# sp-uhh/sgmse

Measured on AMD Instinct MI355X. Metric: utterances/sec, SGMSE+ NCSN++ PC N=30 (reverse_diffusion + ALD, 60 NFE), 16 kHz 4 s utterances, higher is better.
Workload: dtype f32 (fp16x2-split products, fp32 accumulate); 1 GPU; BASELINE configs[1]: ncsnpp (65.6M params) PC sampler N=30, batch=32 x 4 s @16 kHz per GPU, hipGraph-captured step; batch_per_gpu=32, F=256, T=512, nfe=60, sampler=pc, parallelism=utterance-sharded x1 (weights broadcast once over RCCL)

## Files before the change

### include/sgmse_hip.h

```cpp
#ifndef SGMSE_HIP_H
#define SGMSE_HIP_H

#ifdef __cplusplus
extern "C" {
#endif

typedef struct sgmse_ctx sgmse_ctx;

typedef enum { SGMSE_OK = 0, SGMSE_EINVAL = -1, SGMSE_ERUNTIME = -2, SGMSE_ENOTREADY = -3 } sgmse_status;

typedef struct {
  int variant;
  int nf;
  int n_levels;
  int ch_mult[8];
  int num_res_blocks;
  int n_attn;
  int attn_res[8];
  int image_size;
  int progressive;
  int progressive_input;
  int scale_by_sigma;
} sgmse_net_cfg;

// ... 36 lines not shown
int sgmse_stft(sgmse_ctx* ctx, const float* sig, const float* window, void* spec, int B, int L, int n_fft, int hop);
int sgmse_istft(sgmse_ctx* ctx, const void* spec, const float* window, float* out, int B, int K, int n_fft, int hop,
                int length);
int sgmse_spec_fwd(sgmse_ctx* ctx, const void* in, void* out, long long n, int transform_type, float factor, float exponent);
int sgmse_spec_back(sgmse_ctx* ctx, const void* in, void* out, long long n, int transform_type, float factor, float exponent);

int sgmse_upfirdn2d(sgmse_ctx* ctx, const float* input, const float* kernel, float* out, int BC, int H, int W, int kh,
                    int kw, int up_x, int up_y, int down_x, int down_y, int pad_x0, int pad_x1, int pad_y0, int pad_y1);
int sgmse_upfirdn2d_dtype(sgmse_ctx* ctx, int dtype, const void* input, const void* kernel, void* out, int BC, int H, int W,
                          int kh, int kw, int up_x, int up_y, int down_x, int down_y, int pad_x0, int pad_x1, int pad_y0,
                          int pad_y1);

int sgmse_op_conv2d(sgmse_ctx* ctx, const float* x, const float* w_oihw, const float* bias, const float* res, float* out,
                    int B, int Cin, int Cout, int H, int W, int ks, float out_scale, int force_direct,
                    const float* in_scale, const float* in_shift, int in_act, const float* x2, int C2);
int sgmse_op_groupnorm(sgmse_ctx* ctx, const float* x, const float* gamma, const float* beta, float* out, int B, int C,
                       int H, int W, int act, const float* x2, int C2);
int sgmse_op_fir(sgmse_ctx* ctx, const float* x, float* out, int BC, int H, int W, int up, const float* in_scale,
                 const float* in_shift, int in_act, float* out_raw);
int sgmse_op_attention(sgmse_ctx* ctx, const float* qkv, float* out, int B, int C, int S);

int sgmse_conv_split_mode(sgmse_ctx* ctx, int* out);
int sgmse_conv_winograd(sgmse_ctx* ctx, int* out);

#define SGMSE_NCLASS 8
int sgmse_profile_forward(sgmse_ctx* ctx, const void* xy, const float* t, void* out, int B, int F, int T, float* ms,
                          double* work, int* launches);
int sgmse_bench_conv(sgmse_ctx* ctx, int ks, int B, int Cin, int Cout, int H, int W, int variant, int iters, int fused,
                     float* ms);
int sgmse_calib_stream(sgmse_ctx* ctx, int mode, int bytes_per_lane, long long total_bytes, float* ms);
// ... 11 lines not shown
```

### sgmse_amd/_lib.py

```python
from __future__ import annotations

import ctypes as C
import os
import threading
from typing import Dict, Optional, Sequence

import torch

_HERE = os.path.dirname(os.path.abspath(__file__))
DEFAULT_LIB = os.path.join(_HERE, "libsgmse_hip.so")

SGMSE_NCLASS = 8
CLASS_NAMES = ("conv3x3_wide", "conv3x3_other", "conv1x1", "conv_direct", "groupnorm_stats", "fir",
               "attention", "entry_exit")
CLASS_WORK_UNIT = ("flop", "flop", "flop", "flop", "byte", "byte", "flop", "byte")


class NetCfgC(C.Structure):
    _fields_ = [("variant", C.c_int), ("nf", C.c_int), ("n_levels", C.c_int), ("ch_mult", C.c_int * 8),
                ("num_res_blocks", C.c_int), ("n_attn", C.c_int), ("attn_res", C.c_int * 8), ("image_size", C.c_int),
                ("progressive", C.c_int), ("progressive_input", C.c_int), ("scale_by_sigma", C.c_int)]


class SamplerCfgC(C.Structure):
# ... 17 lines not shown
    "sgmse_last_error": (C.c_char_p, [_P]),
    "sgmse_backend": (C.c_char_p, []),
    "sgmse_configure": (_I, [_P, C.POINTER(NetCfgC)]),
    "sgmse_load_weights": (_I, [_P, C.POINTER(C.c_char_p), C.POINTER(_P), C.POINTER(_LL), _I, _I]),
    "sgmse_param_count": (_I, [_P, C.POINTER(_LL)]),
    "sgmse_ncsnpp_forward": (_I, [_P, _P, _P, _P, _I, _I, _I]),
    "sgmse_pc_sample": (_I, [_P, _P, _P, _I, _I, _I, C.POINTER(SamplerCfgC), _P, C.c_ulonglong, C.POINTER(_I)]),
    "sgmse_sb_sample": (_I, [_P, _P, _P, _I, _I, _I, _I] + [C.POINTER(_F)] * 8 + [_I, _P, C.c_ulonglong, _I, C.POINTER(_I)]),
    "sgmse_stft": (_I, [_P, _P, _P, _P, _I, _I, _I, _I]),
    "sgmse_istft": (_I, [_P, _P, _P, _P, _I, _I, _I, _I, _I]),
    "sgmse_spec_fwd": (_I, [_P, _P, _P, _LL, _I, _F, _F]),
    "sgmse_spec_back": (_I, [_P, _P, _P, _LL, _I, _F, _F]),
    "sgmse_upfirdn2d": (_I, [_P, _P, _P, _P] + [_I] * 13),
    "sgmse_upfirdn2d_dtype": (_I, [_P, _I, _P, _P, _P] + [_I] * 13),
    "sgmse_op_conv2d": (_I, [_P, _P, _P, _P, _P, _P, _I, _I, _I, _I, _I, _I, _F, _I, _P, _P, _I, _P, _I]),
    "sgmse_op_groupnorm": (_I, [_P, _P, _P, _P, _P, _I, _I, _I, _I, _I, _P, _I]),
    "sgmse_conv_split_mode": (_I, [_P, _P]),
    "sgmse_conv_winograd": (_I, [_P, _P]),
    "sgmse_op_fir": (_I, [_P, _P, _P, _I, _I, _I, _I, _P, _P, _I, _P]),
    "sgmse_op_attention": (_I, [_P, _P, _P, _I, _I, _I]),
    "sgmse_profile_forward": (_I, [_P, _P, _P, _P, _I, _I, _I, C.POINTER(_F), C.POINTER(C.c_double), C.POINTER(_I)]),
    "sgmse_bench_conv": (_I, [_P, _I, _I, _I, _I, _I, _I, _I, _I, _I, C.POINTER(_F)]),
    "sgmse_calib_stream": (_I, [_P, _I, _I, C.c_longlong, C.POINTER(_F)]),
    "sgmse_arena_bytes": (_I, [_P, C.POINTER(_LL)]),
    "sgmse_graph_captures": (_I, [_P, C.POINTER(_I)]),
    "sgmse_graph_updates": (_I, [_P, C.POINTER(_I)]),
    "sgmse_set_noise_streams": (_I, [_P, C.POINTER(C.c_ulonglong), _I]),
    "sgmse_set_frames": (_I, [_P, C.POINTER(_I), _I]),
}
EXPORTED_SYMBOLS = tuple(_SIGS)
# ... 384 lines not shown
```

### sgmse_amd/csrc/capi.h

```cpp
#pragma once
#include <string>
#include "engine.h"
#include "../../include/sgmse_hip.h"

struct sgmse_ctx {
  sgmse::Engine* eng = nullptr;
  std::string err;
};

namespace {
template <class Fn>
int sg_guard(sgmse_ctx* ctx, Fn&& fn) {
  if (!ctx || !ctx->eng) return SGMSE_EINVAL;
  try {
    fn(*ctx->eng);
    return SGMSE_OK;
  } catch (const sgmse::EngineError& e) {
    ctx->err = e.what();
    const bool notready = ctx->err.find("weights not loaded") != std::string::npos;
    return notready ? SGMSE_ENOTREADY : SGMSE_ERUNTIME;
  } catch (const std::exception& e) {
    ctx->err = std::string("internal error: ") + e.what();
    return SGMSE_ERUNTIME;
  }
// ... 130 lines not shown
  SG_ARG(ctx, up_x >= 1 && up_y >= 1 && down_x >= 1 && down_y >= 1, "up/down factors must be >= 1");
  return sg_guard(ctx, [&](sgmse::Engine& e) { e.op_upfirdn2d(dtype, input, kernel, out, BC, H, W, kh, kw, up_x, up_y, down_x, down_y, px0, px1, py0, py1); });
}

int sgmse_op_conv2d(sgmse_ctx* ctx, const float* x, const float* w, const float* bias, const float* res, float* out, int B, int Cin,
                    int Cout, int H, int W, int ks, float out_scale, int force_direct, const float* in_scale,
                    const float* in_shift, int in_act, const float* x2, int C2) {
  SG_ARG(ctx, x && w && out && B > 0 && Cin > 0 && Cout > 0 && H > 0 && W > 0, "null pointer or non-positive shape");
  SG_ARG(ctx, ks == 1 || ks == 3, "kernel size must be 1 or 3");
  SG_ARG(ctx, (x2 == nullptr) == (C2 == 0) && C2 >= 0 && C2 < Cin, "bad second source");
  return sg_guard(ctx, [&](sgmse::Engine& e) {
    e.op_conv2d(x, w, bias, res, out, B, Cin, Cout, H, W, ks, out_scale, force_direct, in_scale, in_shift, in_act, x2, C2);
  });
}

int sgmse_op_groupnorm(sgmse_ctx* ctx, const float* x, const float* gamma, const float* beta, float* out, int B, int C, int H,
                       int W, int act, const float* x2, int C2) {
  SG_ARG(ctx, x && gamma && beta && out && B > 0 && C >= 4 && H > 0 && W > 0, "null pointer or non-positive shape");
  SG_ARG(ctx, C % (C / 4 < 32 ? C / 4 : 32) == 0, "C must be divisible by min(C/4, 32)");
  return sg_guard(ctx, [&](sgmse::Engine& e) { e.op_groupnorm(x, gamma, beta, out, B, C, H, W, act, x2, C2); });
}

int sgmse_conv_split_mode(sgmse_ctx* ctx, int* out) {
  SG_ARG(ctx, out != nullptr, "out is null");
  return sg_guard(ctx, [&](sgmse::Engine& e) { *out = e.split_mode(); });
}

int sgmse_conv_winograd(sgmse_ctx* ctx, int* out) {
  SG_ARG(ctx, out != nullptr, "out is null");
  return sg_guard(ctx, [&](sgmse::Engine& e) { *out = e.winograd() ? 1 : 0; });
// ... 56 lines not shown
```

### sgmse_amd/csrc/conv_launch.h

```cpp
#pragma once
#include "conv_route.h"
#include "kernels_conv.h"
#include "kernels_conv_pipe.h"
#include "kernels_conv1x1.h"
#include "kernels_conv_split.h"
#include "kernels_conv_wino.h"
#include "kernels_conv_wino43.h"
#include "kernels_conv_wino2d.h"
#include "kernels_conv_thin.h"

#ifndef SGMSE_CONV_SPLIT_DEFAULT
#define SGMSE_CONV_SPLIT_DEFAULT 2
#endif
#ifndef SGMSE_CONV_PIPE_DEFAULT
#define SGMSE_CONV_PIPE_DEFAULT 1
#endif

namespace sgmse {

inline int conv_variant() {
  static int v = [] { const char* e = getenv("SGMSE_CONV_VARIANT"); return e ? atoi(e) : 0; }();
  return v;
}

// ... 101 lines not shown
  if (abl && mode == 2) {
#define SGMSE_ABL_CASE(V) if (abl == V) { DRT_LAUNCH((conv3x3_split_kernel<SplitH2, 0, 1, V>), grid, dim3(256), st, a); return; }
#ifdef SGMSE_ABLATION_FULL
    SGMSE_ABL_CASE(8) SGMSE_ABL_CASE(59) SGMSE_ABL_CASE(64)
    SGMSE_ABL_CASE(3) SGMSE_ABL_CASE(4) SGMSE_ABL_CASE(24) SGMSE_ABL_CASE(56)
    SGMSE_ABL_CASE(1) SGMSE_ABL_CASE(2) SGMSE_ABL_CASE(67) SGMSE_ABL_CASE(72) SGMSE_ABL_CASE(128) SGMSE_ABL_CASE(256) SGMSE_ABL_CASE(512)
#endif
#undef SGMSE_ABL_CASE
  }
  if (mode == 2) launch_conv3x3_split_t<SplitH2, 0>(a, grid, st); else launch_conv3x3_split_t<SplitB3, 0>(a, grid, st);
}

inline bool conv_wino43_aligned(const ConvArgs& a) {
  return reinterpret_cast<uintptr_t>(a.src1) % 16 == 0 && (a.src2 == nullptr || reinterpret_cast<uintptr_t>(a.src2) % 16 == 0);
}
template <int ROWS>
inline void launch_conv_wino_rows(WinoForm form, const ConvArgs& a, drt::stream_t st) {
  const dim3 grid(conv_grid_tiles(a, ROWS), a.Cout / 128, 1);
  const bool act = a.in_scale && a.in_act;
  if (form == WinoForm::F43) {
    if (act) DRT_LAUNCH((conv3x3_wino43_kernel<ROWS, 1>), grid, dim3(512), st, a);
    else DRT_LAUNCH((conv3x3_wino43_kernel<ROWS, 0>), grid, dim3(512), st, a);
  } else {
    if (a.sc_w) DRT_LAUNCH((conv3x3_wino_kernel<ROWS, 1, 1>), grid, dim3(512), st, a);
    else if (act) DRT_LAUNCH((conv3x3_wino_kernel<ROWS, 1, 0>), grid, dim3(512), st, a);
    else DRT_LAUNCH((conv3x3_wino_kernel<ROWS, 0, 0>), grid, dim3(512), st, a);
  }
}
inline void launch_conv_wino(WinoForm form, const ConvArgs& a, drt::stream_t st, bool rows4, bool trace = false, int abl = 0) {
  if (form == WinoForm::F2x2) {
    const dim3 grid(conv_grid_tiles(a, 4), a.Cout / 128, 1);
    if (abl == 8) DRT_LAUNCH((conv3x3_wino2d_kernel<1, 8>), grid, dim3(512), st, a);
    else if (abl == 16) DRT_LAUNCH((conv3x3_wino2d_kernel<1, 16>), grid, dim3(512), st, a);
    else if (a.in_scale && a.in_act) DRT_LAUNCH((conv3x3_wino2d_kernel<1>), grid, dim3(512), st, a);
    else DRT_LAUNCH((conv3x3_wino2d_kernel<0>), grid, dim3(512), st, a);
    return;
  }
#ifdef SGMSE_ABLATION_FULL
  const dim3 grid8(conv_grid_tiles(a, 8), a.Cout / 128, 1);
  if (form == WinoForm::F43) {
    if (trace) { DRT_LAUNCH((conv3x3_wino43_kernel<8, 1, 1>), grid8, dim3(512), st, a); return; }
  } else {
#define SGMSE_WABL_CASE(V) if (abl == V) { DRT_LAUNCH((conv3x3_wino_kernel<8, 1, 0, 0, V>), grid8, dim3(512), st, a); return; }
    SGMSE_WABL_CASE(1) SGMSE_WABL_CASE(2) SGMSE_WABL_CASE(4) SGMSE_WABL_CASE(8) SGMSE_WABL_CASE(16) SGMSE_WABL_CASE(24) SGMSE_WABL_CASE(3) SGMSE_WABL_CASE(32) SGMSE_WABL_CASE(20)
#undef SGMSE_WABL_CASE
    if (trace) { DRT_LAUNCH((conv3x3_wino_kernel<8, 1, 0, 1>), grid8, dim3(512), st, a); return; }
  }
#endif
  (void)abl; (void)trace;
  if (rows4) launch_conv_wino_rows<4>(form, a, st); else launch_conv_wino_rows<8>(form, a, st);
}

inline void launch_conv_thin(const ConvArgs& a, drt::stream_t st) {
  const dim3 grid(conv_thin_grid_tiles(a, (a.W + ConvThinGeom::TW - 1) / ConvThinGeom::TW), 1, 1);
  if (a.in_scale && a.in_act) DRT_LAUNCH((conv3x3_thin_kernel<1>), grid, dim3(256), st, a);
  else DRT_LAUNCH((conv3x3_thin_kernel<0>), grid, dim3(256), st, a);
}

inline void launch_conv_direct(const ConvArgs& a, int ks, drt::stream_t st) {
  const int HW = a.H * a.W;
  if (a.Cout <= 4) {
    dim3 grid((HW + 255) / 256, 1, a.B);
    if (ks == 3) DRT_LAUNCH((conv_direct_kernel<3, 4>), grid, dim3(256), st, a);
    else DRT_LAUNCH((conv_direct_kernel<1, 4>), grid, dim3(256), st, a);
  } else {
// ... 8 lines not shown
```

### sgmse_amd/csrc/engine.h

```cpp
#pragma once
#include <map>
#include <string>
#include <vector>
#include <cstdio>
#include <stdexcept>

#include <deque>
#include <sgmse_devrt.h>
#include "kernels_conv.h"
#include "conv_launch.h"
#include "kernels_norm_fir.h"
#include "kernels_attn_misc.h"
#include "kernels_stft.h"

namespace sgmse {

struct EngineError : std::runtime_error { using std::runtime_error::runtime_error; };

#define SG_CHECK(expr) do { int _e = (expr); if (_e != 0) { char _b[256]; snprintf(_b, sizeof _b, "%s failed: %s (%d)", #expr, drt::error_string(_e), _e); throw EngineError(_b); } } while (0)
#define SG_REQUIRE(cond, msg) do { if (!(cond)) throw EngineError(std::string(msg)); } while (0)

struct NetCfg {
  int variant = 0;
  int nf = 128;
// ... 550 lines not shown
      if (bounds) free_tmp(bounds);
      if (xb) free_tmp(xb);
    } else if (pl.mfma && !force_direct && (C2 == 0 || a.C1 % ((ks == 3) ? 8 : 32) == 0)) {
      const float* pk = pack_mfma(oihw_sources(w_oihw, ks, Cin, Cout), pl.co_t, false);
      a.w = pk;
      launch_conv_mfma(a, ks, pl, stream_);
      SG_CHECK(drt::stream_sync(stream_));
      free_tmp(const_cast<float*>(pk));
    } else {
      a.w = w_oihw;
      launch_conv_direct(a, ks, stream_);
    }
    check_launch();
  }

  void op_groupnorm(const float* x, const float* gamma, const float* beta, float* out, int B, int C, int H, int W, int act,
                    const float* x2, int C2) {
    const int HW = H * W, C1 = C - C2;
    float* stats = static_cast<float*>(dev_alloc_tmp((size_t)B * C * 2 * 4));
    float* sc = static_cast<float*>(dev_alloc_tmp((size_t)B * C * 4));
    float* sh = static_cast<float*>(dev_alloc_tmp((size_t)B * C * 4));
    float* stats2 = stats + (size_t)B * C1 * 2;
    DRT_LAUNCH(gn_chan_stats_kernel, dim3(B * C1), dim3(256), stream_, x, (const float*)nullptr, C1, 0, HW, stats, Rag{nullptr, nullptr, nullptr}, 0);
    if (C2) DRT_LAUNCH(gn_chan_stats_kernel, dim3(B * C2), dim3(256), stream_, x2, (const float*)nullptr, C2, 0, HW, stats2, Rag{nullptr, nullptr, nullptr}, 0);
    const int G = std::min(C / 4, 32);
    const GnFin f{stats, stats2, nullptr, nullptr, gamma, beta, sc, sh, nullptr, Rag{nullptr, nullptr, nullptr}, C1, 1, 1, C2, 1, 1, G, HW, 0, 1e-6f};
    DRT_LAUNCH(gn_finalize_kernel, dim3(G, B), dim3(256), stream_, f);
    DRT_LAUNCH(gn_apply_kernel, dim3((HW + 1023) / 1024, B * C), dim3(256), stream_, x, x2, C1, C2, HW, (const float*)sc,
               (const float*)sh, act, out);
    SG_CHECK(drt::stream_sync(stream_));
// ... 45 lines not shown
  }

  void op_spec_xform(const float2* in, float2* out, size_t n, int type, float factor, float exponent, int inverse) {
    SpecXformArgs a{in, out, n, type, factor, exponent, inverse};
    DRT_LAUNCH(spec_xform_kernel, dim3((unsigned)((n + 255) / 256)), dim3(256), stream_, a);
    check_launch();
  }

  void sync() { SG_CHECK(drt::stream_sync(stream_)); }

  float bench_conv(int ks, int B, int Cin, int Cout, int H, int W, int variant, int iters, int fused) {
    ConvPlan pl = choose_conv_plan(ks, Cin, Cout, H, W);
    SG_REQUIRE(pl.mfma, "bench_conv: shape is not MFMA-eligible");
    if (variant >= 0 && (variant & 512)) { pl.rows = 4; variant &= ~512; }
    int ablate = 0, abl_split = 0;
    bool split_rows4 = false, wino43 = false;
    if (variant >= 0) {
      split_rows4 = (variant >> 23) & 1;
      wino43 = (variant >> 22) & 1;
      abl_split = (variant >> 12) & 1023;
      if (!(variant & (64 | 128))) { ablate = abl_split & 15; abl_split = 0; }
      variant &= 4095;
    }
    const bool wino = variant >= 0 && (variant & 1024);
    const bool wino2d = variant >= 0 && (variant & 2048) && !wino;
    const int smode = variant < 0 ? 0 : ((variant & 128) ? 2 : ((variant & 64) ? 1 : 0));
    const bool b3 = smode != 0 && !wino && !wino2d;
    SG_REQUIRE(!(wino || wino2d) || (ks == 3 && conv_wino_eligible(Cin, 0, Cout, W)), "bench_conv: shape is not eligible for the Winograd kernel");
    SG_REQUIRE(!b3 || conv_split_eligible(ks, Cin, 0, Cout), "bench_conv: shape is not eligible for the split kernels");
    wino43 = wino43 && wino;
    SG_REQUIRE(!wino43 || conv_wino43_eligible(Cin, 0, Cout, W), "bench_conv: shape is not eligible for the Winograd F(4,3) kernel");
    const WinoForm wform = wino2d ? WinoForm::F2x2 : wino43 ? WinoForm::F43 : WinoForm::F23;
// ... 24 lines not shown
          a.in_scale = nullptr; a.in_shift = nullptr; a.in_act = 0;
          a.amax1 = bounds;
        } else {
          xbound = producer_bound(a.in_scale, a.in_shift, Cin, bounds, nullptr, B); a.xbound = xbound;
        }
      }
    }
    unsigned long long* trace_dev = nullptr;
    const size_t n_wg = (size_t)B * ((H + 7) / 8) * ((W + 31) / 32) * ((Cout + 127) / 128);
    if (abl_split & 64) {
      trace_dev = static_cast<unsigned long long*>(dev_alloc_tmp(n_wg * 256));
      SG_CHECK(drt::memset_dev(trace_dev, 0, n_wg * 256, stream_));
      a.trace = trace_dev;
    }
    auto go = [&]() {
      if (wino || wino2d) launch_conv_wino(wform, a, stream_, split_rows4, (abl_split & 64) != 0, abl_split & 63);
      else if (b3) launch_conv_split(a, ks, smode, stream_, split_rows4, abl_split);
      else launch_conv_mfma(a, ks, pl, stream_, variant);
    };
    for (int i = 0; i < 2; ++i) go();
    drt::event_record(&e0, stream_);
    for (int i = 0; i < iters; ++i) go();
    drt::event_record(&e1, stream_);
    drt::event_sync(&e1);
    const float ms = drt::event_elapsed_ms(e0, e1) / (float)iters;
    check_launch();
    drt::event_destroy(&e0); drt::event_destroy(&e1);
    if (trace_dev) {
      const size_t words = wino ? 32 : 16;
      std::vector<unsigned long long> h(n_wg * words);
      SG_CHECK(drt::memcpy_d2h(h.data(), trace_dev, n_wg * words * 8, stream_));
// ... 1044 lines not shown
```

### sgmse_amd/csrc/kernels_conv_wino43.h

```cpp
#pragma once
#include "kernels_conv_wino.h"

namespace sgmse {

template <int ROWS_>
struct Wino43Geom {
  static constexpr int KC = 16, ROWS = ROWS_, TROWS = ROWS_ + 2, NF = ROWS_ / 4, NK = 6;
  static constexpr int PV = 25;
  static constexpr int ROW_V = 8 * PV;
  static constexpr int STAGE_V = TROWS * ROW_V;
  static constexpr int NSROW = 4 * TROWS;
  static constexpr int NPASS = (NSROW + 5) / 6;
  static constexpr int CO_V = 512;
  static constexpr int NDIR = ROWS_ == 4 ? 1 : 2;
  static constexpr int XCH_V = 4 * NDIR * 16 * 64;
  static constexpr int LDS_V = (2 * STAGE_V + CO_V) > XCH_V ? (2 * STAGE_V + CO_V) : XCH_V;
  static_assert(NPASS <= 8, "one staging pass per wave");
};

inline size_t packed_wino43_frags(int cin, int cout) { return (size_t)((cout + 127) / 128) * (cin / 16) * 18 * 2 * 4 * 64; }
inline size_t packed_wino43_bytes(int cin, int cout) { return packed_wino43_frags(cin, cout) * 16 + (size_t)((cout + 127) / 128) * 128 * 4; }

__device__ __forceinline__ double wino43_u(double g0, double g1, double g2, int k) {
  return k == 0 ? 0.25 * g0 : k == 1 ? -(g0 + g1 + g2) / 6.0 : k == 2 ? -(g0 - g1 + g2) / 6.0
// ... 42 lines not shown
      double u = 0.0;
      if (co < p.cout) {
        const float* g = p.src + (((size_t)co * p.cin + c) * 3 + dy) * 3;
        u = wino43_u(g[0], g[1], g[2], k);
      }
      u *= ws;
      const uint32_t hi = drt_f32_to_f16((float)u);
      const uint32_t lo = drt_f32_to_f16((float)(u - (double)drt_f16_to_f32(hi)));
      part[h] = split ? lo : hi;
    }
    o[q] = part[0] | (part[1] << 16);
  }
  reinterpret_cast<u32x4*>(p.dst)[e] = o;
}

template <int ROWS, int ACT, int TRACE = 0>
__global__ __launch_bounds__(512, 1) void conv3x3_wino43_kernel(ConvArgs p) {
  using G = Wino43Geom<ROWS>;
  using T = WinoTile<ROWS>;
  using S = SplitH2;
  constexpr int NF = G::NF, PV = G::PV, NS = 2;
  __shared__ u32x4 s_all[G::LDS_V];
  u32x4* const s_in0 = s_all;
  u32x4* const s_in1 = s_all + G::STAGE_V;
  f32x4* const s_co = reinterpret_cast<f32x4*>(s_all + 2 * G::STAGE_V);

  const int tid = threadIdx.x;
  const int wave = drt_uniform(tid >> 6), lane = tid & 63, l31 = lane & 31, kg = lane >> 5;
  const int cf = wave & 3, kh = wave >> 2;
  unsigned long long* trace = nullptr;
  if constexpr (TRACE) {
// ... 162 lines not shown
  if (it_run) {
#pragma unroll
    for (int c = 0; c < 4; ++c) stage_chan_co(c, s_co[4 * it_q + c]);
    flush_item(s_in0);
    load_item((nst > 1 ? 1 : 0) * G::KC);
  }
  __syncthreads();

  if constexpr (TRACE) { if (trace) trace[2] = drt_clock(); }
  constexpr int AR = 3, AD = AR - 1, NTAP = 9;
  unsigned long long tbar = 0, ttap[NTAP] = {0, 0, 0, 0, 0, 0, 0, 0, 0};
  const bool tracer = TRACE && p.trace && (tid == 0 || tid == 256);
  u32x4 ar[AR][NS];
#pragma unroll
  for (int t = 0; t < AD; ++t) load_a(0, t, ar[t]);
#pragma unroll 1
  for (int st = 0; st < nst; ++st) {
    const int stn = st + 1 < nst ? st + 1 : st;
    const int stl = st + 2 < nst ? st + 2 : nst - 1;
    const u32x4* cur = (st & 1) ? s_in1 : s_in0;
    u32x4* nxt = (st & 1) ? s_in0 : s_in1;
#pragma unroll
    for (int tap = 0; tap < NTAP; ++tap) {
      unsigned long long tc0 = 0;
      if constexpr (TRACE) tc0 = drt_clock();
      const int ntap = (tap + AD) % NTAP;
      const int nstg = tap + AD < NTAP ? st : stn;
      load_a(nstg, ntap, ar[(tap + AD) % AR]);
      __builtin_amdgcn_sched_barrier(0);
      const bool ca = tap < 2, cb = tap >= NTAP - 2;
      const int phase = ca ? tap : cb ? tap - (NTAP - 2) : -1;
      const bool stage_here = phase >= 0 && it_run && (ca ? kh == 0 : kh == 1) && st + 1 < nst;
      compute_tap(cur, tap, ar[tap % AR], phase, stage_here, stn * G::KC, nxt);
      if (phase == 1 && stage_here && st + 2 < nst) load_item(stl * G::KC);
      if constexpr (TRACE) { __builtin_amdgcn_sched_barrier(0); ttap[tap] += drt_clock() - tc0; }
    }
    if constexpr (TRACE) {
      const unsigned long long tb = drt_clock();
      __syncthreads();
      tbar += drt_clock() - tb;
    } else {
      __syncthreads();
    }
  }
  if constexpr (TRACE) {
    if (trace) { trace[3] = drt_clock(); trace[6] = tbar; }
    if (tracer) {
      unsigned long long* tq = p.trace + 32 * (size_t)(blockIdx.y * gridDim.x + blockIdx.x) + (tid == 0 ? 11 : 21);
#pragma unroll
      for (int i = 0; i < NTAP; ++i) tq[i] = ttap[i];
      tq[NTAP] = tbar;
    }
  }

  constexpr bool ALL_TO_A = ROWS == 4;
  const bool fin_wave = !ALL_TO_A || kh == 0;
  const int ef = ALL_TO_A ? 0 : kh;
  int tid_e = (int)threadIdx.x;
  DRT_PIN_INT(tid_e);
  const int lane_e = tid_e & 63, l31_e = lane_e & 31, kg_e = lane_e >> 5;
  const int yy_raw = y0 + 4 * ef + (l31_e >> 3), x = x0 + 4 * (l31_e & 7);
  const bool okc = x < W;
  const bool inside = x0 + 32 <= W && y0 + ROWS <= H;
  const size_t ubase = (size_t)b * p.Cout * HW;
  const int co_l = co_blk * 128 + cf * 32 + 4 * kg_e;
  const int yy = yy_raw < H ? yy_raw : H - 1;
  const unsigned lane_boff = (((unsigned)co_l * (unsigned)H + (unsigned)yy) * (unsigned)W + (unsigned)(okc ? x : 0)) * 4u;
  auto soff = [&](int r) -> unsigned { return (unsigned)((r & 3) + 8 * (r >> 2)) * HW * 4u; };
  const drt_buf obuf = drt_make_buf(p.out + ubase), rbuf = drt_make_buf(p.res ? p.res + ubase : p.out);
  const bool has_res = p.res != nullptr;
  float2 rr[16][2];
  if (fin_wave && has_res) {
#pragma unroll
    for (int r = 0; r < 16; ++r) { rr[r][0] = drt_buf_load2(rbuf, lane_boff, soff(r)); rr[r][1] = drt_buf_load2(rbuf, lane_boff + 8u, soff(r)); }
  }
  if constexpr (TRACE) { if (trace) trace[7] = drt_clock() - trace[3]; }
  float yv[4][16];
  {
    float4* xs = reinterpret_cast<float4*>(s_all);
    auto slot = [&](int dir, int r) -> float4* { return xs + (((cf * G::NDIR + dir) * 16 + r) * 64 + lane_e); };
    auto part_a = [&](int f, int r) -> float4 {
      const float m1 = acc[1][f][r], m2 = acc[2][f][r];
      const float sp = m1 + m2, sm = m1 - m2;
      return make_float4(acc[0][f][r] + sp, sm, sp, sm);
    };
    auto part_b = [&](int f, int r) -> float4 {
      const float m3 = acc[0][f][r], m4 = acc[1][f][r];
      const float s = m3 + m4, t = m3 - m4;
      return make_float4(s, 2.f * t, 4.f * s, 8.f * t + acc[2][f][r]);
    };
    if (kh == 0) {
// ... 25 lines not shown
      }
    }
  }
  if constexpr (TRACE) { if (trace) trace[5] = drt_clock() - trace[3]; }
  auto finish = [&](auto guard_tag) {
    constexpr bool GUARD = decltype(guard_tag)::value;
    float cs_inv[16];
    load_cs(cs_inv);
    float s1[16], s2[16], vmax = 0.f;
    const bool ok = !GUARD || (okc && yy_raw < H);
#pragma unroll
    for (int r = 0; r < 16; ++r) {
      float v[4];
#pragma unroll
      for (int i = 0; i < 4; ++i) v[i] = yv[i][r] * cs_inv[r] * inv_kx;
      if (has_res) { v[0] += rr[r][0].x; v[1] += rr[r][0].y; v[2] += rr[r][1].x; v[3] += rr[r][1].y; }
#pragma unroll
      for (int i = 0; i < 4; ++i) v[i] *= p.out_scale;
      if (ok) {
        drt_buf_store2(obuf, make_float2(v[0], v[1]), lane_boff, soff(r));
        drt_buf_store2(obuf, make_float2(v[2], v[3]), lane_boff + 8u, soff(r));
      }
      if (GUARD) {
#pragma unroll
        for (int i = 0; i < 4; ++i) v[i] = ok ? v[i] : 0.f;
      }
      vmax = fmaxf(fmaxf(vmax, fmaxf(fabsf(v[0]), fabsf(v[1]))), fmaxf(fabsf(v[2]), fabsf(v[3])));
      s1[r] = (v[0] + v[1]) + (v[2] + v[3]);
      s2[r] = (v[0] * v[0] + v[1] * v[1]) + (v[2] * v[2] + v[3] * v[3]);
    }
    DRT_PIN_HERE(vmax);
    if constexpr (TRACE) { if (trace) trace[10] = drt_clock() - trace[3]; }
    if (p.stats_out && y0 + 4 * ef < H) {
      auto butterfly = [&](float (&sv)[16]) -> float {
        float a[8];
#pragma unroll
// ... 28 lines not shown
```

### sgmse_amd/csrc/sgmse_devrt.h

```cpp
#pragma once
#include <hip/hip_runtime.h>
#include <cstdint>
#include <cstddef>
#include <cstdlib>
#include <cstring>
#include <cmath>
#include <algorithm>

typedef float f32x16 __attribute__((ext_vector_type(16)));
typedef float f32x4 __attribute__((ext_vector_type(4)));
typedef float f32x2 __attribute__((ext_vector_type(2)));
typedef uint32_t u32x4 __attribute__((ext_vector_type(4)));

__device__ __forceinline__ f32x16 mfma_32x32x16_bf16(u32x4 a, u32x4 b, f32x16 c) {
  typedef __bf16 bf16x8 __attribute__((ext_vector_type(8)));
  return __builtin_amdgcn_mfma_f32_32x32x16_bf16(__builtin_bit_cast(bf16x8, a), __builtin_bit_cast(bf16x8, b), c, 0, 0, 0);
}

__device__ __forceinline__ f32x16 mfma_32x32x16_f16(u32x4 a, u32x4 b, f32x16 c) {
  typedef _Float16 f16x8 __attribute__((ext_vector_type(8)));
  return __builtin_amdgcn_mfma_f32_32x32x16_f16(__builtin_bit_cast(f16x8, a), __builtin_bit_cast(f16x8, b), c, 0, 0, 0);
}
__device__ __forceinline__ uint32_t drt_f32_to_f16(float x) { return (uint32_t)__builtin_bit_cast(uint16_t, (_Float16)x); }
__device__ __forceinline__ float drt_f16_to_f32(uint32_t h) { return (float)__builtin_bit_cast(_Float16, (uint16_t)h); }
// ... 18 lines not shown
}
template <int AUX = 0>
__device__ __forceinline__ void drt_buf_store(const drt_buf& b, float v, unsigned voff, unsigned soff) {
  __builtin_amdgcn_raw_buffer_store_b32(__builtin_bit_cast(unsigned, v), b.r, voff, soff, AUX);
}
template <int AUX = 0>
__device__ __forceinline__ float2 drt_buf_load2(const drt_buf& b, unsigned voff, unsigned soff) {
  const auto v = __builtin_amdgcn_raw_buffer_load_b64(b.r, voff, soff, AUX);
  return make_float2(__builtin_bit_cast(float, (unsigned)v[0]), __builtin_bit_cast(float, (unsigned)v[1]));
}
template <int AUX = 0>
__device__ __forceinline__ void drt_buf_store2(const drt_buf& b, float2 v, unsigned voff, unsigned soff) {
  typedef unsigned u2_t __attribute__((ext_vector_type(2)));
  const u2_t u = {__builtin_bit_cast(unsigned, v.x), __builtin_bit_cast(unsigned, v.y)};
  __builtin_amdgcn_raw_buffer_store_b64(u, b.r, voff, soff, AUX);
}
__device__ __forceinline__ unsigned long long drt_clock() { return __builtin_amdgcn_s_memtime(); }
__device__ __forceinline__ unsigned drt_hw_id() { return __builtin_amdgcn_s_getreg((31 << 11) | 4); }
__device__ __forceinline__ unsigned drt_xcc_id() { return __builtin_amdgcn_s_getreg((31 << 11) | 20); }
__device__ __forceinline__ void drt_atomic_max_nonneg(float* p, float v) {
  atomicMax(reinterpret_cast<unsigned int*>(p), __builtin_bit_cast(unsigned int, v));
}

__device__ __forceinline__ double drt_shfl_xor_f64(double v, int mask) {
  const unsigned long long u = __builtin_bit_cast(unsigned long long, v);
  const unsigned lo = (unsigned)__shfl_xor((int)(unsigned)(u & 0xffffffffull), mask);
  const unsigned hi = (unsigned)__shfl_xor((int)(unsigned)(u >> 32), mask);
  return __builtin_bit_cast(double, ((unsigned long long)hi << 32) | lo);
}

// ... 106 lines not shown
```

### sgmse_amd/ops.py

```python
from __future__ import annotations

from typing import Dict, Optional, Tuple

import torch

from . import _lib

_ctx: Dict[str, "_lib.Context"] = {}


def default_context(device: "torch.device | str | None" = None) -> "_lib.Context":
    if device is None:
        device = "cpu" if _lib.is_emulator() else torch.device("cuda", torch.cuda.current_device())
    key = str(torch.device(device))
    if key not in _ctx:
        _ctx[key] = _lib.Context(device)
    return _ctx[key]


def _f32(t: Optional[torch.Tensor], name: str, dev) -> Optional[torch.Tensor]:
    return None if t is None else _lib.check_tensor(t, name, torch.float32, dev)


def conv2d(x: torch.Tensor, weight: torch.Tensor, bias: Optional[torch.Tensor] = None, *,
# ... 6 lines not shown
    B, C1, H, W = x.shape
    C2 = 0 if x2 is None else x2.shape[1]
    Cout, Cin, kh, kw = weight.shape
    if kh != kw or kh not in (1, 3):
        raise ValueError("kernel must be 1x1 or 3x3")
    if Cin != C1 + C2:
        raise ValueError(f"weight expects {Cin} input channels, got {C1}+{C2}")
    out = torch.empty((B, Cout, H, W), dtype=torch.float32, device=dev)
    ctx.use_current_stream()
    ctx.check(ctx.lib.sgmse_op_conv2d(ctx.h, x.data_ptr(), weight.data_ptr(), _lib.ptr(_f32(bias, "bias", dev)),
                                      _lib.ptr(_f32(residual, "residual", dev)), out.data_ptr(), B, Cin, Cout, H, W, kh,
                                      float(out_scale), {None: int(force_direct), 'bf16x3': 2, 'fp16x2': 3, 'wino': 4, 'wino4': 5, 'thin': 6, 'wino2d': 7, 'wino43': 8, 'wino43_4': 9}[force_split], _lib.ptr(_f32(in_scale, "in_scale", dev)),
                                      _lib.ptr(_f32(in_shift, "in_shift", dev)), int(in_act),
                                      _lib.ptr(_f32(x2, "x2", dev)), C2))
    return out


def group_norm(x: torch.Tensor, weight: torch.Tensor, bias: torch.Tensor, *, act: bool = False,
               x2: Optional[torch.Tensor] = None) -> torch.Tensor:
    ctx = default_context(x.device)
    dev = ctx.device
    x = _f32(x, "x", dev)
    B, C1, H, W = x.shape
    C2 = 0 if x2 is None else x2.shape[1]
    C = C1 + C2
    out = torch.empty((B, C, H, W), dtype=torch.float32, device=dev)
    ctx.use_current_stream()
    ctx.check(ctx.lib.sgmse_op_groupnorm(ctx.h, x.data_ptr(), _f32(weight, "weight", dev).data_ptr(),
                                         _f32(bias, "bias", dev).data_ptr(), out.data_ptr(), B, C, H, W, int(act),
                                         _lib.ptr(_f32(x2, "x2", dev)), C2))
# ... 96 lines not shown
```

Measured before the change: 6.140 utterances/s.

## Overlap Winograd F(4,3) residual loads with last stage and widen epilogue stores

Peels the last K-stage of the Winograd F(4,3) conv main loop so that residual loads are issued during its later taps, hiding their latency behind the MFMA work instead of loading after the loop. The epilogue now loads and stores 128-bit values when output and residual are 16-byte aligned, replacing pairs of 64-bit buffer ops. The old path stays available as the EPI8 template variant and is used as a fallback for unaligned cases. It also adds a standalone op and C API for testing the kernel. Holding the residual in 16 float4 registers during the last stage raises register pressure, which could hurt the schedule.

```diff
diff --git a/include/sgmse_hip.h b/include/sgmse_hip.h
--- a/include/sgmse_hip.h
+++ b/include/sgmse_hip.h
@@ -74,6 +74,9 @@
 int sgmse_op_conv2d(sgmse_ctx* ctx, const float* x, const float* w_oihw, const float* bias, const float* res, float* out,
                     int B, int Cin, int Cout, int H, int W, int ks, float out_scale, int force_direct,
                     const float* in_scale, const float* in_shift, int in_act, const float* x2, int C2);
+int sgmse_op_conv_wino43(sgmse_ctx* ctx, const float* x, const float* w_oihw, const float* bias, const float* res, float* out,
+                         float* stats_out, float* amax_out, const float* xbound, int B, int Cin, int Cout, int H, int W, float out_scale,
+                         const float* in_scale, const float* in_shift, int in_act, const int* frames, int rows4, int epi8);
 int sgmse_op_groupnorm(sgmse_ctx* ctx, const float* x, const float* gamma, const float* beta, float* out, int B, int C,
                        int H, int W, int act, const float* x2, int C2);
 int sgmse_op_fir(sgmse_ctx* ctx, const float* x, float* out, int BC, int H, int W, int up, const float* in_scale,
diff --git a/sgmse_amd/_lib.py b/sgmse_amd/_lib.py
--- a/sgmse_amd/_lib.py
+++ b/sgmse_amd/_lib.py
@@ -55,6 +55,7 @@
     "sgmse_upfirdn2d": (_I, [_P, _P, _P, _P] + [_I] * 13),
     "sgmse_upfirdn2d_dtype": (_I, [_P, _I, _P, _P, _P] + [_I] * 13),
     "sgmse_op_conv2d": (_I, [_P, _P, _P, _P, _P, _P, _I, _I, _I, _I, _I, _I, _F, _I, _P, _P, _I, _P, _I]),
+    "sgmse_op_conv_wino43": (_I, [_P] * 9 + [_I] * 5 + [_F, _P, _P, _I, _P, _I, _I]),
     "sgmse_op_groupnorm": (_I, [_P, _P, _P, _P, _P, _I, _I, _I, _I, _I, _P, _I]),
     "sgmse_conv_split_mode": (_I, [_P, _P]),
     "sgmse_conv_winograd": (_I, [_P, _P]),
diff --git a/sgmse_amd/csrc/capi.h b/sgmse_amd/csrc/capi.h
--- a/sgmse_amd/csrc/capi.h
+++ b/sgmse_amd/csrc/capi.h
@@ -168,6 +168,16 @@
   });
 }
 
+int sgmse_op_conv_wino43(sgmse_ctx* ctx, const float* x, const float* w, const float* bias, const float* res, float* out, float* stats_out,
+                         float* amax_out, const float* xbound, int B, int Cin, int Cout, int H, int W, float out_scale,
+                         const float* in_scale, const float* in_shift, int in_act, const int* frames, int rows4, int epi8) {
+  SG_ARG(ctx, x && w && out && stats_out && amax_out && xbound && B > 0 && Cin > 0 && Cout > 0 && H > 0 && W > 0, "null pointer or non-positive shape");
+  SG_ARG(ctx, (in_scale == nullptr) == (in_shift == nullptr), "in_scale and in_shift come together");
+  return sg_guard(ctx, [&](sgmse::Engine& e) {
+    e.op_conv_wino43(x, w, bias, res, out, stats_out, amax_out, xbound, B, Cin, Cout, H, W, out_scale, in_scale, in_shift, in_act, frames, rows4, epi8);
+  });
+}
+
 int sgmse_op_groupnorm(sgmse_ctx* ctx, const float* x, const float* gamma, const float* beta, float* out, int B, int C, int H,
                        int W, int act, const float* x2, int C2) {
   SG_ARG(ctx, x && gamma && beta && out && B > 0 && C >= 4 && H > 0 && W > 0, "null pointer or non-positive shape");
diff --git a/sgmse_amd/csrc/conv_launch.h b/sgmse_amd/csrc/conv_launch.h
--- a/sgmse_amd/csrc/conv_launch.h
+++ b/sgmse_amd/csrc/conv_launch.h
@@ -139,20 +139,29 @@
 inline bool conv_wino43_aligned(const ConvArgs& a) {
   return reinterpret_cast<uintptr_t>(a.src1) % 16 == 0 && (a.src2 == nullptr || reinterpret_cast<uintptr_t>(a.src2) % 16 == 0);
 }
+inline bool conv_wino43_epilogue_aligned(const ConvArgs& a) {
+  return reinterpret_cast<uintptr_t>(a.out) % 16 == 0 && (a.res == nullptr || reinterpret_cast<uintptr_t>(a.res) % 16 == 0) &&
+         (a.rag_w ? a.rag_vec_ok != 0 : a.W % 4 == 0);
+}
 template <int ROWS>
-inline void launch_conv_wino_rows(WinoForm form, const ConvArgs& a, drt::stream_t st) {
+inline void launch_conv_wino_rows(WinoForm form, const ConvArgs& a, drt::stream_t st, bool epi8) {
   const dim3 grid(conv_grid_tiles(a, ROWS), a.Cout / 128, 1);
   const bool act = a.in_scale && a.in_act;
   if (form == WinoForm::F43) {
-    if (act) DRT_LAUNCH((conv3x3_wino43_kernel<ROWS, 1>), grid, dim3(512), st, a);
-    else DRT_LAUNCH((conv3x3_wino43_kernel<ROWS, 0>), grid, dim3(512), st, a);
+    if (epi8 || !conv_wino43_epilogue_aligned(a)) {
+      if (act) DRT_LAUNCH((conv3x3_wino43_kernel<ROWS, 1, 0, 1>), grid, dim3(512), st, a);
+      else DRT_LAUNCH((conv3x3_wino43_kernel<ROWS, 0, 0, 1>), grid, dim3(512), st, a);
+    } else {
+      if (act) DRT_LAUNCH((conv3x3_wino43_kernel<ROWS, 1>), grid, dim3(512), st, a);
+      else DRT_LAUNCH((conv3x3_wino43_kernel<ROWS, 0>), grid, dim3(512), st, a);
+    }
   } else {
     if (a.sc_w) DRT_LAUNCH((conv3x3_wino_kernel<ROWS, 1, 1>), grid, dim3(512), st, a);
     else if (act) DRT_LAUNCH((conv3x3_wino_kernel<ROWS, 1, 0>), grid, dim3(512), st, a);
     else DRT_LAUNCH((conv3x3_wino_kernel<ROWS, 0, 0>), grid, dim3(512), st, a);
   }
 }
-inline void launch_conv_wino(WinoForm form, const ConvArgs& a, drt::stream_t st, bool rows4, bool trace = false, int abl = 0) {
+inline void launch_conv_wino(WinoForm form, const ConvArgs& a, drt::stream_t st, bool rows4, bool trace = false, int abl = 0, bool epi8 = false) {
   if (form == WinoForm::F2x2) {
     const dim3 grid(conv_grid_tiles(a, 4), a.Cout / 128, 1);
     if (abl == 8) DRT_LAUNCH((conv3x3_wino2d_kernel<1, 8>), grid, dim3(512), st, a);
@@ -164,6 +173,7 @@
 #ifdef SGMSE_ABLATION_FULL
   const dim3 grid8(conv_grid_tiles(a, 8), a.Cout / 128, 1);
   if (form == WinoForm::F43) {
+    if (trace && epi8) { DRT_LAUNCH((conv3x3_wino43_kernel<8, 1, 1, 1>), grid8, dim3(512), st, a); return; }
     if (trace) { DRT_LAUNCH((conv3x3_wino43_kernel<8, 1, 1>), grid8, dim3(512), st, a); return; }
   } else {
 #define SGMSE_WABL_CASE(V) if (abl == V) { DRT_LAUNCH((conv3x3_wino_kernel<8, 1, 0, 0, V>), grid8, dim3(512), st, a); return; }
@@ -173,7 +183,7 @@
   }
 #endif
   (void)abl; (void)trace;
-  if (rows4) launch_conv_wino_rows<4>(form, a, st); else launch_conv_wino_rows<8>(form, a, st);
+  if (rows4) launch_conv_wino_rows<4>(form, a, st, epi8); else launch_conv_wino_rows<8>(form, a, st, epi8);
 }
 
 inline void launch_conv_thin(const ConvArgs& a, drt::stream_t st) {
diff --git a/sgmse_amd/csrc/engine.h b/sgmse_amd/csrc/engine.h
--- a/sgmse_amd/csrc/engine.h
+++ b/sgmse_amd/csrc/engine.h
@@ -588,6 +588,48 @@
     check_launch();
   }
 
+  void op_conv_wino43(const float* x, const float* w_oihw, const float* bias, const float* res, float* out, float* stats_out, float* amax_out,
+                      const float* xbound, int B, int Cin, int Cout, int H, int W, float out_scale, const float* in_scale, const float* in_shift,
+                      int in_act, const int* frames, int rows4, int epi8) {
+    ConvArgs a{};
+    a.src1 = x; a.C1 = Cin; a.bias = bias; a.res = res; a.out_scale = out_scale; a.out = out; a.Cout = Cout; a.B = B; a.H = H; a.W = W;
+    a.in_scale = in_scale; a.in_shift = in_shift; a.in_act = in_act; a.xbound = xbound;
+    SG_REQUIRE(conv_wino43_eligible(Cin, 0, Cout, W) && conv_wino43_aligned(a), "op_conv_wino43: shape is not eligible for the Winograd F(4,3) kernel");
+    a.stats_out = stats_out; a.stats_rows = 4; a.stats_nsub = ((H + 3) / 4) * ((W + 31) / 32);
+    a.amax_out = amax_out;
+    SG_CHECK(drt::memset_dev(amax_out, 0, (size_t)B * kAmaxSpread * 4, stream_));
+    void* rag = nullptr;
+    if (frames) {
+      SG_REQUIRE(H % 4 == 0, "op_conv_wino43: a ragged batch needs H % 4 == 0");
+      std::vector<long long> tab(3 * (size_t)(B + 1), 0);
+      long long *off = tab.data(), *soff = off + (B + 1);
+      int* wc = reinterpret_cast<int*>(soff + (B + 1));
+      int* cols = wc + B;
+      cols[0] = 0;
+      for (int b = 0; b < B; ++b) {
+        SG_REQUIRE(frames[b] > 0 && frames[b] <= W && frames[b] % 4 == 0, "op_conv_wino43: widths must be multiples of 4 and at most W");
+        wc[b] = frames[b];
+        off[b + 1] = off[b] + (long long)H * frames[b];
+        soff[b + 1] = soff[b] + (long long)H * ((frames[b] + 31) / 32);
+        cols[b + 1] = cols[b] + (frames[b] + 31) / 32;
+      }
+      rag = dev_alloc_tmp(tab.size() * 8);
+      SG_CHECK(drt::memcpy_h2d(rag, tab.data(), tab.size() * 8, stream_));
+      SG_CHECK(drt::stream_sync(stream_));
+      long long* d = static_cast<long long*>(rag);
+      a.rag_off = d; a.rag_soff = d + (B + 1);
+      a.rag_w = reinterpret_cast<const int*>(d + 2 * (B + 1)); a.rag_cols = a.rag_w + B; a.rag_ncols = cols[B];
+      a.rag_vec_ok = 1;
+    }
+    const float* pk = pack_wino(WinoForm::F43, w_oihw, Cin, Cout, false, &a.co_scale);
+    a.w = pk;
+    launch_conv_wino(WinoForm::F43, a, stream_, rows4 != 0, false, 0, epi8 != 0);
+    SG_CHECK(drt::stream_sync(stream_));
+    free_tmp(const_cast<float*>(pk));
+    if (rag) free_tmp(rag);
+    check_launch();
+  }
+
   void op_groupnorm(const float* x, const float* gamma, const float* beta, float* out, int B, int C, int H, int W, int act,
                     const float* x2, int C2) {
     const int HW = H * W, C1 = C - C2;
@@ -663,8 +705,9 @@
     SG_REQUIRE(pl.mfma, "bench_conv: shape is not MFMA-eligible");
     if (variant >= 0 && (variant & 512)) { pl.rows = 4; variant &= ~512; }
     int ablate = 0, abl_split = 0;
-    bool split_rows4 = false, wino43 = false;
+    bool split_rows4 = false, wino43 = false, epi8 = false;
     if (variant >= 0) {
+      epi8 = (variant >> 24) & 1;
       split_rows4 = (variant >> 23) & 1;
       wino43 = (variant >> 22) & 1;
       abl_split = (variant >> 12) & 1023;
@@ -719,7 +762,7 @@
       a.trace = trace_dev;
     }
     auto go = [&]() {
-      if (wino || wino2d) launch_conv_wino(wform, a, stream_, split_rows4, (abl_split & 64) != 0, abl_split & 63);
+      if (wino || wino2d) launch_conv_wino(wform, a, stream_, split_rows4, (abl_split & 64) != 0, abl_split & 63, epi8);
       else if (b3) launch_conv_split(a, ks, smode, stream_, split_rows4, abl_split);
       else launch_conv_mfma(a, ks, pl, stream_, variant);
     };
diff --git a/sgmse_amd/csrc/kernels_conv_wino43.h b/sgmse_amd/csrc/kernels_conv_wino43.h
--- a/sgmse_amd/csrc/kernels_conv_wino43.h
+++ b/sgmse_amd/csrc/kernels_conv_wino43.h
@@ -1,5 +1,18 @@
 #pragma once
 #include "kernels_conv_wino.h"
+
+#ifdef SGMSE_EMULATOR
+template <int AUX = 0>
+static inline float4 drt_buf_load4(const drt_buf& b, unsigned voff, unsigned soff) {
+  const float2 lo = drt_buf_load2<AUX>(b, voff, soff), hi = drt_buf_load2<AUX>(b, voff + 8u, soff);
+  return make_float4(lo.x, lo.y, hi.x, hi.y);
+}
+template <int AUX = 0>
+static inline void drt_buf_store4(const drt_buf& b, float4 v, unsigned voff, unsigned soff) {
+  drt_buf_store2<AUX>(b, make_float2(v.x, v.y), voff, soff);
+  drt_buf_store2<AUX>(b, make_float2(v.z, v.w), voff + 8u, soff);
+}
+#endif
 
 namespace sgmse {
 
@@ -80,7 +93,7 @@
   reinterpret_cast<u32x4*>(p.dst)[e] = o;
 }
 
-template <int ROWS, int ACT, int TRACE = 0>
+template <int ROWS, int ACT, int TRACE = 0, int EPI8 = 0>
 __global__ __launch_bounds__(512, 1) void conv3x3_wino43_kernel(ConvArgs p) {
   using G = Wino43Geom<ROWS>;
   using T = WinoTile<ROWS>;
@@ -273,8 +286,17 @@
   u32x4 ar[AR][NS];
 #pragma unroll
   for (int t = 0; t < AD; ++t) load_a(0, t, ar[t]);
-#pragma unroll 1
-  for (int st = 0; st < nst; ++st) {
+  float4 rr[16];
+  auto soff = [&](int r) -> unsigned { return (unsigned)((r & 3) + 8 * (r >> 2)) * HW * 4u; };
+  unsigned long long t_res = 0;
+  constexpr int RES_LAST = NTAP - 1 - AD;
+#ifndef SGMSE_WINO43_RES_FROM
+#define SGMSE_WINO43_RES_FROM 6
+#endif
+  constexpr int RES_FROM = SGMSE_WINO43_RES_FROM;
+  static_assert(RES_FROM >= 0 && RES_FROM <= RES_LAST, "residual loads go out behind a live weight load of the last stage");
+  auto run_stage = [&](int st, auto last_tag, const drt_buf* rbuf_l, unsigned lane_boff_l, bool res_l) {
+    constexpr bool LAST = decltype(last_tag)::value;
     const int stn = st + 1 < nst ? st + 1 : st;
     const int stl = st + 2 < nst ? st + 2 : nst - 1;
     const u32x4* cur = (st & 1) ? s_in1 : s_in0;
@@ -285,13 +307,21 @@
       if constexpr (TRACE) tc0 = drt_clock();
       const int ntap = (tap + AD) % NTAP;
       const int nstg = tap + AD < NTAP ? st : stn;
-      load_a(nstg, ntap, ar[(tap + AD) % AR]);
+      if (!LAST || tap + AD < NTAP) load_a(nstg, ntap, ar[(tap + AD) % AR]);
+      if constexpr (LAST) {
+        if (tap >= RES_FROM && tap <= RES_LAST && res_l) {
+          constexpr int NT = RES_LAST - RES_FROM + 1;
+#pragma unroll
+          for (int r = 16 * (tap - RES_FROM) / NT; r < 16 * (tap - RES_FROM + 1) / NT; ++r) rr[r] = drt_buf_load4(*rbuf_l, lane_boff_l, soff(r));
+        }
+        if constexpr (TRACE) { if (tap == RES_LAST) t_res = drt_clock(); }
+      }
       __builtin_amdgcn_sched_barrier(0);
       const bool ca = tap < 2, cb = tap >= NTAP - 2;
       const int phase = ca ? tap : cb ? tap - (NTAP - 2) : -1;
-      const bool stage_here = phase >= 0 && it_run && (ca ? kh == 0 : kh == 1) && st + 1 < nst;
-      compute_tap(cur, tap, ar[tap % AR], phase, stage_here, stn * G::KC, nxt);
-      if (phase == 1 && stage_here && st + 2 < nst) load_item(stl * G::KC);
+      const bool stage_here = !LAST && phase >= 0 && it_run && (ca ? kh == 0 : kh == 1) && st + 1 < nst;
+      compute_tap(cur, tap, ar[tap % AR], LAST ? -1 : phase, stage_here, stn * G::KC, nxt);
+      if (!LAST && phase == 1 && stage_here && st + 2 < nst) load_item(stl * G::KC);
       if constexpr (TRACE) { __builtin_amdgcn_sched_barrier(0); ttap[tap] += drt_clock() - tc0; }
     }
     if constexpr (TRACE) {
@@ -301,16 +331,10 @@
     } else {
       __syncthreads();
     }
-  }
-  if constexpr (TRACE) {
-    if (trace) { trace[3] = drt_clock(); trace[6] = tbar; }
-    if (tracer) {
-      unsigned long long* tq = p.trace + 32 * (size_t)(blockIdx.y * gridDim.x + blockIdx.x) + (tid == 0 ? 11 : 21);
-#pragma unroll
-      for (int i = 0; i < NTAP; ++i) tq[i] = ttap[i];
-      tq[NTAP] = tbar;
-    }
-  }
+  };
+  const int nloop = EPI8 ? nst : nst - 1;
+#pragma unroll 1
+  for (int st = 0; st < nloop; ++st) run_stage(st, std::false_type{}, nullptr, 0u, false);
 
   constexpr bool ALL_TO_A = ROWS == 4;
   const bool fin_wave = !ALL_TO_A || kh == 0;
@@ -325,15 +349,31 @@
   const int co_l = co_blk * 128 + cf * 32 + 4 * kg_e;
   const int yy = yy_raw < H ? yy_raw : H - 1;
   const unsigned lane_boff = (((unsigned)co_l * (unsigned)H + (unsigned)yy) * (unsigned)W + (unsigned)(okc ? x : 0)) * 4u;
-  auto soff = [&](int r) -> unsigned { return (unsigned)((r & 3) + 8 * (r >> 2)) * HW * 4u; };
   const drt_buf obuf = drt_make_buf(p.out + ubase), rbuf = drt_make_buf(p.res ? p.res + ubase : p.out);
   const bool has_res = p.res != nullptr;
-  float2 rr[16][2];
-  if (fin_wave && has_res) {
-#pragma unroll
-    for (int r = 0; r < 16; ++r) { rr[r][0] = drt_buf_load2(rbuf, lane_boff, soff(r)); rr[r][1] = drt_buf_load2(rbuf, lane_boff + 8u, soff(r)); }
-  }
-  if constexpr (TRACE) { if (trace) trace[7] = drt_clock() - trace[3]; }
+  const bool res_here = fin_wave && has_res;
+  if constexpr (!EPI8) run_stage(nst - 1, std::true_type{}, &rbuf, lane_boff, res_here);
+  if constexpr (TRACE) {
+    if (trace) { trace[3] = drt_clock(); trace[6] = tbar; }
+    if (tracer) {
+      unsigned long long* tq = p.trace + 32 * (size_t)(blockIdx.y * gridDim.x + blockIdx.x) + (tid == 0 ? 11 : 21);
+#pragma unroll
+      for (int i = 0; i < NTAP; ++i) tq[i] = ttap[i];
+      tq[NTAP] = tbar;
+    }
+  }
+
+  if constexpr (EPI8) {
+    if (res_here) {
+#pragma unroll
+      for (int r = 0; r < 16; ++r) {
+        const float2 lo = drt_buf_load2(rbuf, lane_boff, soff(r)), hi = drt_buf_load2(rbuf, lane_boff + 8u, soff(r));
+        rr[r] = make_float4(lo.x, lo.y, hi.x, hi.y);
+      }
+    }
+    if constexpr (TRACE) t_res = drt_clock();
+  }
+  if constexpr (TRACE) { if (trace) trace[7] = t_res - trace[3]; }
   float yv[4][16];
   {
     float4* xs = reinterpret_cast<float4*>(s_all);
@@ -389,12 +429,16 @@
       float v[4];
 #pragma unroll
       for (int i = 0; i < 4; ++i) v[i] = yv[i][r] * cs_inv[r] * inv_kx;
-      if (has_res) { v[0] += rr[r][0].x; v[1] += rr[r][0].y; v[2] += rr[r][1].x; v[3] += rr[r][1].y; }
+      if (has_res) { v[0] += rr[r].x; v[1] += rr[r].y; v[2] += rr[r].z; v[3] += rr[r].w; }
 #pragma unroll
       for (int i = 0; i < 4; ++i) v[i] *= p.out_scale;
       if (ok) {
-        drt_buf_store2(obuf, make_float2(v[0], v[1]), lane_boff, soff(r));
-        drt_buf_store2(obuf, make_float2(v[2], v[3]), lane_boff + 8u, soff(r));
+        if constexpr (EPI8) {
+          drt_buf_store2(obuf, make_float2(v[0], v[1]), lane_boff, soff(r));
+          drt_buf_store2(obuf, make_float2(v[2], v[3]), lane_boff + 8u, soff(r));
+        } else {
+          drt_buf_store4(obuf, make_float4(v[0], v[1], v[2], v[3]), lane_boff, soff(r));
+        }
       }
       if (GUARD) {
 #pragma unroll
diff --git a/sgmse_amd/csrc/sgmse_devrt.h b/sgmse_amd/csrc/sgmse_devrt.h
--- a/sgmse_amd/csrc/sgmse_devrt.h
+++ b/sgmse_amd/csrc/sgmse_devrt.h
@@ -56,6 +56,17 @@
   typedef unsigned u2_t __attribute__((ext_vector_type(2)));
   const u2_t u = {__builtin_bit_cast(unsigned, v.x), __builtin_bit_cast(unsigned, v.y)};
   __builtin_amdgcn_raw_buffer_store_b64(u, b.r, voff, soff, AUX);
+}
+template <int AUX = 0>
+__device__ __forceinline__ float4 drt_buf_load4(const drt_buf& b, unsigned voff, unsigned soff) {
+  const auto v = __builtin_amdgcn_raw_buffer_load_b128(b.r, voff, soff, AUX);
+  return make_float4(__builtin_bit_cast(float, (unsigned)v[0]), __builtin_bit_cast(float, (unsigned)v[1]),
+                     __builtin_bit_cast(float, (unsigned)v[2]), __builtin_bit_cast(float, (unsigned)v[3]));
+}
+template <int AUX = 0>
+__device__ __forceinline__ void drt_buf_store4(const drt_buf& b, float4 v, unsigned voff, unsigned soff) {
+  const u32x4 u = {__builtin_bit_cast(unsigned, v.x), __builtin_bit_cast(unsigned, v.y), __builtin_bit_cast(unsigned, v.z), __builtin_bit_cast(unsigned, v.w)};
+  __builtin_amdgcn_raw_buffer_store_b128(u, b.r, voff, soff, AUX);
 }
 __device__ __forceinline__ unsigned long long drt_clock() { return __builtin_amdgcn_s_memtime(); }
 __device__ __forceinline__ unsigned drt_hw_id() { return __builtin_amdgcn_s_getreg((31 << 11) | 4); }
diff --git a/sgmse_amd/ops.py b/sgmse_amd/ops.py
--- a/sgmse_amd/ops.py
+++ b/sgmse_amd/ops.py
@@ -44,6 +44,34 @@
                                       _lib.ptr(_f32(in_shift, "in_shift", dev)), int(in_act),
                                       _lib.ptr(_f32(x2, "x2", dev)), C2))
     return out
+
+
+def conv_wino43(x, weight: torch.Tensor, bias: Optional[torch.Tensor], xbound: torch.Tensor, *, residual=None, out_scale: float = 1.0,
+                in_scale: Optional[torch.Tensor] = None, in_shift: Optional[torch.Tensor] = None, in_act: bool = False, H: Optional[int] = None,
+                frames=None, rows4: bool = False, epi8: bool = False):
+    ctx = default_context(x.device)
+    dev = ctx.device
+    x = _f32(x, "x", dev); weight = _f32(weight, "weight", dev)
+    Cout, Cin = weight.shape[:2]
+    if frames is None:
+        B, _, H, W = x.shape
+        npix, nsub = B * H * W, B * ((H + 3) // 4) * ((W + 31) // 32)
+        shape = (B, Cout, H, W)
+    else:
+        B, W = len(frames), max(frames)
+        npix, nsub = sum(H * f for f in frames), sum(H // 4 * ((f + 31) // 32) for f in frames)
+        shape = (Cout * npix,)
+    out = torch.empty(shape, dtype=torch.float32, device=dev)
+    stats = torch.zeros((Cout * nsub, 2), dtype=torch.float32, device=dev)
+    amax = torch.zeros((B, 64), dtype=torch.float32, device=dev)
+    xb = _f32(xbound.reshape(B, 1).repeat(1, 64).contiguous(), "xbound", dev)
+    fr = None if frames is None else (_lib.C.c_int * B)(*frames)
+    ctx.use_current_stream()
+    ctx.check(ctx.lib.sgmse_op_conv_wino43(ctx.h, x.data_ptr(), weight.data_ptr(), _lib.ptr(_f32(bias, "bias", dev)),
+                                           _lib.ptr(_f32(residual, "residual", dev)), out.data_ptr(), stats.data_ptr(), amax.data_ptr(),
+                                           xb.data_ptr(), B, Cin, Cout, H, W, float(out_scale), _lib.ptr(_f32(in_scale, "in_scale", dev)),
+                                           _lib.ptr(_f32(in_shift, "in_shift", dev)), int(in_act), fr, int(rows4), int(epi8)))
+    return out, stats, amax
 
 
 def group_norm(x: torch.Tensor, weight: torch.Tensor, bias: torch.Tensor, *, act: bool = False,
```

After: 6.138 utterances/s. No clear change (-0.0%).
